# liquidcronos/Drone-stabilisation-using-Optical-Flow-Gps-and-Inertial-Sensors

Measured on AMD Instinct MI355X. Metric: frame-pairs/sec @1920x1080 (LK+velocity), higher is better.
Workload: dtype u8/i32 image stages, f32 LK solve, f64 velocity solve; 1 GPU; 1920x1080 frame pairs, 500 Shi-Tomasi corners, 3-level LK pyramid (BASELINE configs[1]); streams_per_gpu=1, win=15, max_level=3

## Files before the change

drone-stabilisation-using-optical-flow-gps-and-inertial-sensors_amd/csrc/k_corners.hip:

```cpp
#include "ofk_internal.h"
#include <type_traits>

__device__ __forceinline__ int reflect101(int i, int n)
{
    if (n == 1) return 0;
    while (i < 0 || i >= n) i = i < 0 ? -i : 2 * (n - 1) - i;
    return i;
}

#define ME_OW 64
#define ME_CAND_MAX 1920

__device__ __forceinline__ int hs_phys(int x) { return (x & ~7) | ((x & 7) ^ ((x >> 3) & 7)); }

template <int BS, bool FUSED>
__global__ __launch_bounds__(256) void k_mineig(const uint8_t *__restrict__ gray, size_t gray_stride, int h, int w,
                                                int bs_rt, int OH, float kd, float ko, float *__restrict__ eig,
                                                size_t eig_stride, unsigned int *__restrict__ maxbits,
                                                const uint8_t *__restrict__ mask, size_t mask_stride, double quality,
                                                unsigned long long *__restrict__ cand, int cand_cap,
                                                int *__restrict__ cand_count, int *__restrict__ flags)
{
    extern __shared__ __attribute__((aligned(16))) uint8_t smem[];
    const int bs = BS ? BS : bs_rt;
// ... 510 lines not shown
    apc = a + c;
    return __float_as_int(apc - sqrt_rn_normal(__builtin_fmaf(4.f, y2, amc2)));
}

#define OFK_PAIR_SPILL_KEYS()                                                                                          \
    {                                                                                                                  \
        const int nchunk = cnt >> 6;                                                                                   \
        for (int q = 0; q < nchunk; ++q) {                                                                             \
            const unsigned long long key = buf[q * 64 + lane];                                                         \
            if (written + q * 64 + lane < seg_cap) myseg[written + q * 64 + lane] = key;                               \
        }                                                                                                              \
        written += nchunk * 64;                                                                                        \
        const unsigned long long rest = buf[nchunk * 64 + lane];                                                       \
        __builtin_amdgcn_wave_barrier();                                                                               \
        buf[lane] = rest;                                                                                              \
        cnt -= nchunk * 64;                                                                                            \
    }
#define OFK_RING_READ(i)                                                                                               \
        const auto oyye = s_ring[(4 * (i)) * 64 + lane], oyyo = s_ring[(4 * (i) + 1) * 64 + lane];                     \
        const auto oxye = s_ring[(4 * (i) + 2) * 64 + lane], oxyo = s_ring[(4 * (i) + 3) * 64 + lane];
#define OFK_PAIR_ROWS(IN)                                                                                             \
    _Pragma("unroll") for (int i = 0; i < BS; ++i) {                                                                   \
        const int r = base + i;                                                                                        \
        int ge2 = (int)__builtin_amdgcn_ubfe((unsigned)curv[i], bsh, 8u), go2 = (int)__builtin_amdgcn_ubfe((unsigned)curv[i], bsh + 8u, 8u); \
        if (!(IN)) {                                                                                                   \
            if (edge_strip) { ge2 = __builtin_amdgcn_ds_bpermute(mir_e, ge2); go2 = __builtin_amdgcn_ds_bpermute(mir_o, go2); } \
        }                                                                                                              \
        if (i > 0 && (i & 1) == 0 && cnt >= 64) OFK_PAIR_SPILL_KEYS()                                                  \
        OFK_RING_READ(i)                                            \
        const int r12e = g1e + ge2, r12o = g1o + go2;               \
        const int se = r01e + r12e, so = r01o + r12o, te = r12e - r01e, to = r12o - r01o;    \
        const int nso = -so, nse = -se, tt = te + to;                                                                  \
        const int dxe = DPP_SHR1(nso) + so;                                                                            \
        const int dxo = DPP_SHL1(se) + nse;                                                                            \
        int uye = DPP_SHR1(to) + te, uyo = DPP_SHL1(te) + to;    \
        asm("" : "+v"(uye), "+v"(uyo));                                \
        const int dye = uye + tt;                                                                                      \
        const int dyo = uyo + tt;                                                                                      \
        int hxxe, hxxo, hxye, hxyo, hyye, hyyo;                                                                        \
        int pxxe = __mul24(dxe, dxe), pyye = __mul24(dye, dye), pxye = __mul24(dxe, dye);                          \
        int pxxo = __mul24(dxo, dxo), pyyo = __mul24(dyo, dyo), pxyo = __mul24(dxo, dyo);                          \
        asm("" : "+v"(pxxe), "+v"(pxye), "+v"(pyye), "+v"(pxxo), "+v"(pxyo), "+v"(pyyo));                          \
        if (!(IN)) {                                                                                               \
            const int Y = Yp0 + r - 2;                                                                             \
            const bool rowflip = (Y < 0) | (Y >= h);                                                               \
            pxye = (rowflip != flip_e) ? -pxye : pxye;                                                             \
            pxyo = (rowflip != flip_o) ? -pxyo : pxyo;                                                             \
        }                                                                                                          \
        box_pair<BS / 2>(pxxe, pxxo, ad2, ad3, hxxe, hxxo);                                                        \
        box_pair<BS / 2>(pxye, pxyo, ad2, ad3, hxye, hxyo);                                                        \
        box_pair<BS / 2>(pyye, pyyo, ad2, ad3, hyye, hyyo);                                                        \
        vxxe += hxxe - rxxe[i]; vxye += hxye - oxye; vyye += hyye - oyye;                                              \
        vxxo += hxxo - rxxo[i]; vxyo += hxyo - oxyo; vyyo += hyyo - oyyo;                                              \
        rxxe[i] = hxxe; rxxo[i] = hxxo;                                                                                \
        s_ring[(4 * i) * 64 + lane] = hyye; s_ring[(4 * i + 1) * 64 + lane] = hyyo;                                    \
        s_ring[(4 * i + 2) * 64 + lane] = hxye; s_ring[(4 * i + 3) * 64 + lane] = hxyo;                                \
        const int yo = ya - 2 + r - BS;                                                                                \
        const int e2e = lambda_min_bits(vxxe, vxye, vyye, kdv), e2o = lambda_min_bits(vxxo, vxyo, vyyo, kdv);    \
        OFK_PAIR_ROW_TAIL(IN)                                                                                          \
        r01e = r12e; r01o = r12o; g1e = ge2; g1o = go2;                                                                  \
    }
#define OFK_PAIR_ROWS_F32(IN)                                                                                          \
    _Pragma("unroll") for (int i = 0; i < BS; ++i) {                                                                   \
        const int r = base + i;                                                                                        \
        const unsigned gw_ = (unsigned)curv[i] >> bsh;                                                                 \
        float ge2 = (float)(gw_ & 255u), go2 = (float)((gw_ >> 8) & 255u);                                             \
        asm("" : "+v"(ge2), "+v"(go2));                   \
        if (!(IN)) {                                                                                                   \
            if (edge_strip) { ge2 = bperm_f(mir_e, ge2); go2 = bperm_f(mir_o, go2); }                                   \
        }                                                                                                              \
        if (i > 0 && (i & 1) == 0 && cnt >= 64) OFK_PAIR_SPILL_KEYS()                                                  \
        OFK_RING_READ(i)                                                                                               \
        const float r12e = g1e + ge2, r12o = g1o + go2;                                                                \
        const float se = r01e + r12e, so = r01o + r12o, te = r12e - r01e, to = r12o - r01o, tt = te + to;              \
        float dxe = so - DPP_SHR1F(so), dxo = DPP_SHL1F(se) - se;                                                      \
        const float dye = (DPP_SHR1F(to) + te) + tt, dyo = (DPP_SHL1F(te) + to) + tt;                                  \
        if (!(IN)) {                                                                                                   \
            const int Y = Yp0 + r - 2;                                                                                 \
            const bool rowflip = (Y < 0) | (Y >= h);                                                                   \
            dxe = (rowflip != flip_e) ? -dxe : dxe;                                                                    \
            dxo = (rowflip != flip_o) ? -dxo : dxo;                                                                    \
        }                                                                                                              \
        const float gx = bperm_f(adk, dxo), gy = bperm_f(adk, dyo);                                                    \
        float hxxe, hxxo, hxye, hxyo, hyye, hyyo;                                                                      \
        const float pxxe = dxe * dxe, pxye = dxe * dye, pyye = dye * dye;                                              \
        box_pair_f<BS / 2>(pxxe, __builtin_fmaf(dxo, dxo, pxxe), gx, gx, ad2, hxxe, hxxo);                              \
        box_pair_f<BS / 2>(pxye, __builtin_fmaf(dxo, dyo, pxye), gx, gy, ad2, hxye, hxyo);                              \
        box_pair_f<BS / 2>(pyye, __builtin_fmaf(dyo, dyo, pyye), gy, gy, ad2, hyye, hyyo);                              \
// ... 24 lines not shown
        const int hm2e = max(max(DPP_SHR1(e2o), e2e), e2o);                                                         \
        const int hm2o = max(max(DPP_SHL1(e2e), e2o), e2e);                                                         \
        const int yn = yo - 1;                                                                                         \
        const int me = max(max(hm0e, hm1e), hm2e), mo = max(max(hm0o, hm1o), hm2o);                                    \
        bool ise = e1e >= max(me, thr1e), iso = e1o >= max(mo, thr1o);                                                 \
        if (!(IN)) {                                                                                                   \
            const bool rnms = (yn >= ya) & (yn < yb) & (yn >= 1) & (yn < h - 1);                                       \
            ise = ise & rnms; iso = iso & rnms;                                                                        \
        }                                                                                                              \
        if (MASK) {                                                                                                    \
            const uint8_t *mrow = mk + (size_t)min(max(yn, 0), h - 1) * w;                                             \
            ise = ise & (mrow[xoc_e] != 0); iso = iso & (mrow[xoc_o] != 0);                                            \
        }                                                                                                              \
        const unsigned long long bale = __builtin_amdgcn_ballot_w64(ise), balo = __builtin_amdgcn_ballot_w64(iso);     \
        const int ne = (int)__popcll(bale);                                                                            \
        OFK_PAIR_KEY_STORE()                                                                                           \
        cnt += ne + (int)__popcll(balo);                                                                               \
        e1e = e2e; e1o = e2o; hm0e = hm1e; hm0o = hm1o; hm1e = hm2e; hm1o = hm2o;

template <int BS> struct pair_geom {
    static constexpr int AN = BS / 2, PAD = (2 + AN + 3) & ~3, D = PAD - 2 - AN, SW = (125 - BS) & ~3;
};

template <int BS, bool MASK>
__global__ __launch_bounds__(64) __attribute__((amdgpu_waves_per_eu(3, 8))) void k_mineig_pair(
    const uint8_t *__restrict__ gray, size_t gray_stride, int h, int w, int rows_per_strip, float kd, float ko,
    unsigned int *__restrict__ maxbits, const uint8_t *__restrict__ mask, size_t mask_stride, double quality,
    unsigned long long *__restrict__ seg, int seg_cap, int *__restrict__ seg_count, int *__restrict__ flags)
{
    static_assert(BS == 3 || BS == 5 || BS == 7, "pair sums are written for odd boxes up to 7");
    constexpr int AN = pair_geom<BS>::AN, PAD = pair_geom<BS>::PAD, D = pair_geom<BS>::D, SW = pair_geom<BS>::SW;
    constexpr int L0 = (BS + 1) / 2, L1 = (BS + 1 + SW) / 2;
    constexpr int NBUF = 64 + 2 * SW;
    __shared__ unsigned long long s_buf[NBUF + 64];
    __shared__ int s_ring_mem[4 * BS * 64];
    const int lane = threadIdx.x;
    int bxi = blockIdx.x, byi = blockIdx.y, b = blockIdx.z;
    if ((gridDim.z & 7) == 0) {
        const unsigned per = gridDim.x * gridDim.y, n = blockIdx.z * per + blockIdx.y * gridDim.x + blockIdx.x, k = n >> 3, rem = k % per;
        b = 8 * (int)(k / per) + (int)(n & 7);
        byi = (int)(rem / gridDim.x); bxi = (int)(rem % gridDim.x);
    }
    const int sx = bxi;
    if (sx * SW - D >= w) return;
    const int ya = byi * rows_per_strip, yb = min(h, ya + rows_per_strip);
    const uint8_t *img = gray + (size_t)b * gray_stride;
    const uint8_t *mk = MASK ? mask + (size_t)b * mask_stride : nullptr;
    unsigned long long *buf = s_buf;

    const int G0 = sx * SW - PAD;
    const int ce = G0 + 2 * lane;
    const bool edge_strip = G0 < 0 || G0 + 128 > w;
    const bool flip_e = ce < 0 || ce >= w, flip_o = ce + 1 < 0 || ce + 1 >= w;
    const int xo_e = ce - (BS - 1) + AN, xo_o = xo_e + 1;
    const bool lane_ok = lane >= L0 && lane < L1;
    const bool own_e = lane_ok && xo_e >= 0 && xo_e < w, own_o = lane_ok && xo_o >= 0 && xo_o < w;
    const bool nms_e = lane_ok && xo_e >= 1 && xo_e < w - 1, nms_o = lane_ok && xo_o >= 1 && xo_o < w - 1;
    const int xoc_e = min(max(xo_e, 0), w - 1), xoc_o = min(max(xo_o, 0), w - 1);

    const int Yp0 = ya - 1 - AN;
    const int nsteps = (yb - ya) + BS + 3;
    const int nstrips = (w + D + SW - 1) / SW;
    const int nseg = nstrips * (int)gridDim.y, segid = byi * nstrips + sx;
    unsigned long long *myseg = seg + ((size_t)b * nseg + segid) * seg_cap;

    const int lrow = lane >> 5, lk = lane & 31;
    const unsigned ldoff = (unsigned)min(max(G0 + 4 * lk, 0), w - 4);
    const int srcsel = (lane >> 1) * 4;
    const unsigned bsh = (unsigned)(lane & 1) * 16u;
    auto mirror = [&](int c) -> int { c = c < 0 ? -c : c; c = c >= w ? 2 * (w - 1) - c : c; return min(max((c - G0) >> 1, 0), 63) * 4; };
    const int mir_e = mirror(ce), mir_o = mirror(ce + 1);
    const int ad2 = ((lane - 2) & 63) * 4, ad3 = ((lane - 3) & 63) * 4;
    constexpr int NL = (BS + 1) / 2;
    auto row_of = [&](int r) -> int {
        int gy = Yp0 - 1 + min(r, nsteps - 1);
        gy = gy < 0 ? -gy : gy;
        return gy >= h ? 2 * (h - 1) - gy : gy;
    };
#define OFK_PAIR_LOAD(R0, OUT)                                                                                         \
    _Pragma("unroll") for (int q_ = 0; q_ < NL; ++q_) {                                                                \
        const unsigned a_ = (unsigned)row_of((R0) + 2 * q_) * (unsigned)w, b_ = (unsigned)row_of((R0) + 2 * q_ + 1) * (unsigned)w; \
        OUT[q_] = (int)*reinterpret_cast<const unsigned *>(img + ((lrow ? b_ : a_) + ldoff));                          \
    }

    float kdv = kd;
    asm volatile("" : "+v"(kdv));
    const int adk = ((lane - AN) & 63) * 4;
    const float lim = kd * 16776960.f;
    auto march = [&](auto fp) -> bool {
        constexpr bool FP = decltype(fp)::value;
        using T = typename std::conditional<FP, float, int>::type;
        T *const s_ring = reinterpret_cast<T *>(s_ring_mem);
        int written = 0, cnt = 0;
        int lmaxi = 0;
        float published = 0.f;
        unsigned mb_seen = __hip_atomic_load(maxbits + b * OFK_MAX_STRIDE, __ATOMIC_RELAXED, __HIP_MEMORY_SCOPE_AGENT);
        float thr = (float)((double)__uint_as_float(mb_seen) * quality);
        T r01e = 0, r01o = 0, g1e = 0, g1o = 0;
        T rxxe[BS], rxxo[BS];
#pragma unroll
        for (int i = 0; i < BS; ++i) { rxxe[i] = rxxo[i] = 0; }
#pragma unroll
        for (int i = 0; i < 4 * BS; ++i) s_ring[i * 64 + lane] = 0;
        T vxxe = 0, vxye = 0, vyye = 0, vxxo = 0, vxyo = 0, vyyo = 0;
        int e1e = 0, e1o = 0, hm0e = 0, hm0o = 0, hm1e = 0, hm1o = 0;
        unsigned long long inexact = 0;
        int nextg[NL];
        OFK_PAIR_LOAD(0, nextg)

        for (int base = 0; base < nsteps; base += BS) {
            int curv[BS];
#pragma unroll
            for (int i = 0; i < BS; ++i) curv[i] = __builtin_amdgcn_ds_bpermute(srcsel + 128 * (i & 1), nextg[i >> 1]);
            if constexpr (FP) {
                if (inexact) return false;
            }
            {
                unsigned cur_seen = (unsigned)__builtin_amdgcn_readfirstlane((int)mb_seen);
                if (__float_as_uint(published) > cur_seen) cur_seen = __float_as_uint(published);
                thr = (float)((double)__uint_as_float(cur_seen) * quality);
            }
            if (cnt >= 64) {
                OFK_PAIR_SPILL_KEYS()
                const float mw = wave_max_f32(lane_ok ? __int_as_float(lmaxi) : 0.f);
                if (mw > published) {
                    if (lane == 0) (void)atomicMax(maxbits + b * OFK_MAX_STRIDE, __float_as_uint(mw));
                    published = mw;
                }
                mb_seen = __hip_atomic_load(maxbits + b * OFK_MAX_STRIDE, __ATOMIC_RELAXED, __HIP_MEMORY_SCOPE_AGENT);
            }
            OFK_PAIR_LOAD(base + BS, nextg)
            const int r1 = base + BS - 1;
            const bool interior = !edge_strip && Yp0 + base - 2 >= 0 && Yp0 + r1 - 2 < h && base >= BS + 3 && ya - 3 + base - BS >= 1 &&
                                  ya - 2 + r1 - BS < yb && ya - 3 + r1 - BS < h - 1;
            const int thrb = __float_as_int(fmaxf(thr, 0.f)) + 1;
            const int thr1e = nms_e ? thrb : 0x7fffffff, thr1o = nms_o ? thrb : 0x7fffffff;
            if constexpr (FP) {
                if (interior) { OFK_PAIR_ROWS_F32(true) } else { OFK_PAIR_ROWS_F32(false) }
            } else {
                if (interior) { OFK_PAIR_ROWS(true) } else { OFK_PAIR_ROWS(false) }
            }
        }
        if constexpr (FP) {
            if (inexact) return false;
        }
        __builtin_amdgcn_wave_barrier();
        for (int i = lane; i < cnt; i += 64)
            if (written + i < seg_cap) myseg[written + i] = buf[i];
        if (lane == 0) {
            seg_count[(size_t)b * nseg + segid] = min(written + cnt, seg_cap);
            if (written + cnt > seg_cap) (void)atomicOr(flags, 1);
        }
        const float mw = wave_max_f32(lane_ok ? __int_as_float(lmaxi) : 0.f);
        if (lane == 0 && mw > published) (void)atomicMax(maxbits + b * OFK_MAX_STRIDE, __float_as_uint(mw));
        return true;
    };
    if (!march(std::true_type{})) march(std::false_type{});
}

#undef OFK_PAIR_LOAD
#undef OFK_PAIR_ROWS
#undef OFK_PAIR_ROWS_F32
#undef OFK_PAIR_ROW_TAIL
#undef OFK_RING_READ
#undef OFK_PAIR_SPILL_KEYS
#undef OFK_LOAD_BLOCK
#undef OFK_EIG_ROWS

static bool pair_ok(int w, int block)
{
    return !g_ofk_tuning.no_pair && (block == 3 || block == 5 || block == 7) && (w & 3) == 0 && w >= 64;
}
static void pair_sw(int block, int *sw, int *d)
{
    switch (block) {
        case 3: *sw = pair_geom<3>::SW; *d = pair_geom<3>::D; break;
        case 5: *sw = pair_geom<5>::SW; *d = pair_geom<5>::D; break;
        default: *sw = pair_geom<7>::SW; *d = pair_geom<7>::D; break;
    }
}

void ofk_stream_geometry(int h, int w, int block, int batch, int *rows, int *nseg, int *seg_cap)
{
// ... 15 lines not shown
{
    constexpr int SW = 61 - BS;
    int rows, nseg, seg_cap;
    ofk_stream_geometry(h, w, BS, batch, &rows, &nseg, &seg_cap);
    if ((size_t)nseg * seg_cap > seg_keys_per_image || nseg > seg_count_cap) return -1;
    const int strips = (w + SW - 1) / SW;
    const double scale = 1.0 / (4.0 * BS * 255.0);
    const float kd = (float)(0.5 * scale * scale), ko = (float)(scale * scale);
    dim3 grid(strips, (h + rows - 1) / rows, batch);
    if (mask)
        hipLaunchKernelGGL((k_mineig_stream<BS, true>), grid, dim3(256 / 4), 0, s, gray, gray_stride, h, w, rows, kd, ko, maxbits, mask,
                           mask_stride, quality, seg, seg_cap, seg_count, flags);
    else
        hipLaunchKernelGGL((k_mineig_stream<BS, false>), grid, dim3(256 / 4), 0, s, gray, gray_stride, h, w, rows, kd, ko, maxbits, mask,
                           mask_stride, quality, seg, seg_cap, seg_count, flags);
    *nseg_out = nseg; *segcap_out = seg_cap;
    return 0;
}

template <int BS>
static int launch_mineig_pair(hipStream_t s, const uint8_t *gray, size_t gray_stride, int h, int w, unsigned int *maxbits,
                              const uint8_t *mask, size_t mask_stride, double quality, unsigned long long *seg,
                              size_t seg_keys_per_image, int *seg_count, int seg_count_cap, int *flags, int batch, int *nseg_out,
                              int *segcap_out)
{
    constexpr int SW = pair_geom<BS>::SW, D = pair_geom<BS>::D;
    int rows, nseg, seg_cap;
    ofk_stream_geometry(h, w, BS, batch, &rows, &nseg, &seg_cap);
    if ((size_t)nseg * seg_cap > seg_keys_per_image || nseg > seg_count_cap) return -1;
    const int strips = (w + D + SW - 1) / SW;
    const double scale = 1.0 / (4.0 * BS * 255.0);
    const float kd = (float)(0.5 * scale * scale), ko = (float)(scale * scale);
    if (ko != 2.f * kd) return -1;
    dim3 grid(strips, (h + rows - 1) / rows, batch);
    if (mask)
        hipLaunchKernelGGL((k_mineig_pair<BS, true>), grid, dim3(64), 0, s, gray, gray_stride, h, w, rows, kd, ko, maxbits, mask,
                           mask_stride, quality, seg, seg_cap, seg_count, flags);
    else
        hipLaunchKernelGGL((k_mineig_pair<BS, false>), grid, dim3(64), 0, s, gray, gray_stride, h, w, rows, kd, ko, maxbits, mask,
                           mask_stride, quality, seg, seg_cap, seg_count, flags);
    *nseg_out = nseg; *segcap_out = seg_cap;
    return 0;
}

int ofk_launch_mineig_cand(hipStream_t s, const uint8_t *gray, size_t gray_stride, int h, int w, int block,
                           unsigned int *maxbits, const uint8_t *mask, size_t mask_stride, double quality,
                           unsigned long long *cand, int cand_cap, int *cand_count, unsigned long long *seg,
                           size_t seg_keys_per_image, int *seg_count, int seg_count_cap, int *flags, int batch, int *nseg_out,
                           int *segcap_out)
{
    *nseg_out = 0; *segcap_out = 0;
#define ME_ARGS s, gray, gray_stride, h, w, block, nullptr, 0, maxbits, mask, mask_stride, quality, cand, cand_cap, cand_count, flags, batch
#define ST_ARGS s, gray, gray_stride, h, w, maxbits, mask, mask_stride, quality, seg, seg_keys_per_image, seg_count, seg_count_cap, flags, batch, nseg_out, segcap_out
    if (pair_ok(w, block)) {
        switch (block) {
            case 3: return launch_mineig_pair<3>(ST_ARGS);
            case 5: return launch_mineig_pair<5>(ST_ARGS);
            default: return launch_mineig_pair<7>(ST_ARGS);
        }
    }
    switch (block) {
        case 3: return launch_mineig_stream<3>(ST_ARGS);
        case 5: return launch_mineig_stream<5>(ST_ARGS);
        case 7: return launch_mineig_stream<7>(ST_ARGS);
        case 12: return launch_mineig_stream<12>(ST_ARGS);
        default: return launch_mineig_t<0, true>(ME_ARGS);
    }
#undef ST_ARGS
#undef ME_ARGS
}

__global__ __launch_bounds__(256) void k_maxbits(const float *__restrict__ eig, size_t eig_stride,
                                                 const uint8_t *__restrict__ mask, size_t mask_stride, int npx,
                                                 unsigned int *__restrict__ maxbits)
{
    const int b = blockIdx.y;
    const float *e = eig + (size_t)b * eig_stride;
    const uint8_t *mk = mask ? mask + (size_t)b * mask_stride : nullptr;
    float m = 0.f;
    for (int i = blockIdx.x * 256 + threadIdx.x; i < npx; i += gridDim.x * 256)
        if (!mk || mk[i]) m = fmaxf(m, e[i]);
// ... 527 lines not shown
```

drone-stabilisation-using-optical-flow-gps-and-inertial-sensors_amd/csrc/ofk_api.hip:

```cpp
#include "ofk_internal.h"
#include <cmath>
#include <stdarg.h>
#include <stdio.h>
#include <stdlib.h>
#include <string.h>

static char g_create_err[512] = "";

int ofk_fail(ofk_ctx *ctx, int code, const char *fmt, ...)
{
    char *dst = ctx ? ctx->errmsg : g_create_err;
    va_list ap;
    va_start(ap, fmt);
    vsnprintf(dst, 512, fmt, ap);
    va_end(ap);
    return code;
}

#define TRY(expr) do { int rc_ = (expr); if (rc_ != OFK_OK) return rc_; } while (0)
static size_t up(size_t v, size_t a) { return (v + a - 1) / a * a; }

ofk_levels ofk_make_levels(int h, int w, int win, int max_level)
{
    ofk_levels lv;
// ... 114 lines not shown
    c->lk_seed_mode = OFK_SEED_OFF; c->lk_seed_gain = 1.0;
    c->robust = ofk_robust{OFK_ROBUST_OFF, 4.685, 5, 64, 0ull, 0};
    c->gate = ofk_track_gate{OFK_FB_OFF, 0.5, -1, 0.0};
    bool ok = hipEventCreateWithFlags(&c->ev_fork, hipEventDisableTiming) == hipSuccess &&
              hipEventCreateWithFlags(&c->ev_x, hipEventDisableTiming) == hipSuccess;
    for (int k = 0; k < OFK_MAX_STREAMS && ok; ++k)
        ok = hipEventCreateWithFlags(&c->ev_g0[k], hipEventDisableTiming) == hipSuccess &&
             hipEventCreateWithFlags(&c->ev_aux[k], hipEventDisableTiming) == hipSuccess &&
             hipEventCreateWithFlags(&c->ev_lkdone[0][k], hipEventDisableTiming) == hipSuccess &&
             hipEventCreateWithFlags(&c->ev_lkdone[1][k], hipEventDisableTiming) == hipSuccess &&
             hipEventCreateWithFlags(&c->ev_end[k], hipEventDisableTiming) == hipSuccess &&
             hipEventCreateWithFlags(&c->ev_stagger[k], hipEventDisableTiming) == hipSuccess;
    if (!ok) {
        ofk_fail(nullptr, OFK_E_HIP, "hipEventCreate failed");
        ofk_destroy(c);
        return OFK_E_HIP;
    }
    const size_t B = (size_t)max_batch;
    for (int k = 0; k < 2; ++k) { ALLOC(c->bgr[k], B * c->bgr_stride); ALLOC(c->pyr[k], B * c->pyr_stride); }
    ALLOC(c->eig, B * c->img_stride * sizeof(float));
    ALLOC(c->cand, B * (size_t)c->cand_cap * 8);
    c->seg_keys = (size_t)(c->P / 4) + (size_t)(c->P / 4) / 2 + 64 * OFK_SEG_MAX;
    ALLOC(c->cand_seg, B * c->seg_keys * 8);
    ALLOC(c->seg_count, B * OFK_SEG_MAX * 4);
    ALLOC(c->cand_count, B * OFK_CNT_STRIDE * 4); ALLOC(c->maxbits, B * OFK_MAX_STRIDE * 4);
    ALLOC(c->sel_hist, B * 1024 * 4);
    ALLOC(c->sel_keys, B * OFK_CHUNK * 8);
    ALLOC(c->pts_prev, B * max_pts * 8); ALLOC(c->pts_next, B * max_pts * 8);
    ALLOC(c->status, B * max_pts); ALLOC(c->err, B * max_pts * 4); ALLOC(c->counts, B * 4);
    ALLOC(c->sensors, B * OFK_SENSOR_DOUBLES * 8); ALLOC(c->records, B * OFK_RECORD_DOUBLES * 8);
    ALLOC(c->dev_flags, 16);
    hipMemsetAsync(c->dev_flags, 0, 16, c->stream);
    hipMemsetAsync(c->counts, 0, B * 4, c->stream);
    hipMemsetAsync(c->sensors, 0, B * OFK_SENSOR_DOUBLES * 8, c->stream);
    c->ev_cap = 32768;
    c->ev = (hipEvent_t *)calloc(c->ev_cap, sizeof(hipEvent_t));
    c->ev_stage = (int *)calloc(c->ev_cap / 2, sizeof(int));
    hipStreamSynchronize(c->stream);
    *out = c;
    return OFK_OK;
}

extern "C" int ofk_destroy(ofk_ctx *c)
{
    if (!c) return OFK_OK;
    hipSetDevice(c->device);
    if (c->stream) hipDeviceSynchronize();
    ofk_comm_destroy(c);
    for (int k = 0; k < 2; ++k) { if (c->bgr[k]) hipFree(c->bgr[k]); if (c->pyr[k]) hipFree(c->pyr[k]); }
    void *ptrs[] = {c->eig, c->mask, c->deriv, c->cand, c->cand_seg, c->seg_count, c->cand_count, c->sel_hist, c->sel_keys, c->maxbits, c->pts_prev, c->pts_next, c->status, c->err,
                    c->counts, c->sensors, c->records, c->dev_flags, c->scratch, c->pts_new, c->new_counts, c->limit,
                    c->imu_state, c->imu_dv, c->kf_mats, c->kf_x, c->kf_P, c->fused, c->imu_msgs, c->imu_counts, c->rob_work, c->pts_back};
    for (void *p : ptrs) if (p) hipFree(p);
    if (c->hstage) hipHostFree(c->hstage);
    ofk_jpeg_release(c);
    if (c->ev) { for (int i = 0; i < c->ev_cap; ++i) if (c->ev[i]) hipEventDestroy(c->ev[i]); free(c->ev); }
    free(c->ev_stage);
    free(c->h_counts);
    for (int k = 1; k < OFK_MAX_STREAMS; ++k) if (c->streams[k]) hipStreamDestroy(c->streams[k]);
    for (int k = 0; k < OFK_MAX_STREAMS; ++k) {
        if (c->aux[k]) hipStreamDestroy(c->aux[k]);
        if (c->ev_g0[k]) hipEventDestroy(c->ev_g0[k]);
        if (c->ev_aux[k]) hipEventDestroy(c->ev_aux[k]);
        for (int s = 0; s < 2; ++s) if (c->ev_lkdone[s][k]) hipEventDestroy(c->ev_lkdone[s][k]);
    }
    for (int k = 0; k < 2; ++k) if (c->pyr_alt[k]) hipFree(c->pyr_alt[k]);
    for (int k = 0; k < 8; ++k) if (c->marks[k]) hipEventDestroy(c->marks[k]);
    for (int k = 0; k < OFK_MAX_STREAMS; ++k) {
        if (c->ev_end[k]) hipEventDestroy(c->ev_end[k]);
        if (c->ev_stagger[k]) hipEventDestroy(c->ev_stagger[k]);
    }
    if (c->ev_x) hipEventDestroy(c->ev_x);
    if (c->ev_fork) hipEventDestroy(c->ev_fork);
// ... 163 lines not shown
    TRY(check_geom(c, batch, h, w, "ofk_mineig_response"));
    if (!gray || !eig) return ofk_fail(c, OFK_E_INVALID, "ofk_mineig_response: NULL buffer");
    TRY(check_block(c, h, w, block));
    const size_t px = (size_t)h * w;
    TRY(h2d(c, c->pyr[0], c->pyr_stride, gray, px, batch));
    if (ofk_launch_mineig(c->stream, c->pyr[0], c->pyr_stride, h, w, block, c->eig, c->img_stride, nullptr, nullptr, 0, batch))
        return ofk_fail(c, OFK_E_INVALID, "k_mineig: LDS tile too large for block_size %d", block);
    TRY(check_launch(c, "k_mineig"));
    return d2h(c, eig, c->eig, c->img_stride * 4, px * 4, batch);
}

static int check_select(ofk_ctx *c, int max_corners, double quality, double min_distance)
{
    if (max_corners < 1 || max_corners > c->max_pts) return ofk_fail(c, OFK_E_INVALID, "max_corners %d outside 1..%d", max_corners, c->max_pts);
    if (!(quality > 0.0) || !(min_distance >= 0.0)) return ofk_fail(c, OFK_E_INVALID, "quality must be > 0 and min_distance >= 0");
    return OFK_OK;
}

static uint8_t *const *pyr_set(ofk_ctx *c, int set) { return set ? c->pyr_alt : c->pyr; }

struct View {
    int nb;
    uint8_t *bgr[2], *pyr[2];
    unsigned int *maxbits; int *cand_count; unsigned long long *cand, *cand_seg; int *seg_count;
    int nseg, segcap;
    unsigned *sel_hist; unsigned long long *sel_keys;
    float *pts_prev, *pts_next; uint8_t *status; float *err; int *counts;
    double *sensors, *records;
    float *pts_back, *err_back, *fb2; uint8_t *status_back; int *gate_stats;
};
static View view_of(ofk_ctx *c, int b0, int nb, int set)
{
    const size_t b = (size_t)b0;
    uint8_t *const *pyr = pyr_set(c, set);
    View v;
    v.nb = nb;
    for (int k = 0; k < 2; ++k) { v.bgr[k] = c->bgr[k] + b * c->bgr_stride; v.pyr[k] = pyr[k] + b * c->pyr_stride; }
    v.maxbits = c->maxbits + b * OFK_MAX_STRIDE; v.cand_count = c->cand_count + b * OFK_CNT_STRIDE;
    v.cand = c->cand + b * c->cand_cap; v.cand_seg = c->cand_seg + b * c->seg_keys; v.seg_count = c->seg_count + b * OFK_SEG_MAX;
    v.nseg = v.segcap = 0;
    v.sel_hist = c->sel_hist + b * 1024; v.sel_keys = c->sel_keys + b * OFK_CHUNK;
    v.pts_prev = c->pts_prev + b * c->max_pts * 2; v.pts_next = c->pts_next + b * c->max_pts * 2;
    v.status = c->status + b * c->max_pts; v.err = c->err + b * c->max_pts; v.counts = c->counts + b;
    v.sensors = c->sensors + b * OFK_SENSOR_DOUBLES; v.records = c->records + b * OFK_RECORD_DOUBLES;
    v.pts_back = v.err_back = v.fb2 = nullptr; v.status_back = nullptr; v.gate_stats = nullptr;
    if (c->pts_back) {
        v.pts_back = c->pts_back + b * c->max_pts * 2; v.err_back = c->err_back + b * c->max_pts; v.fb2 = c->fb2 + b * c->max_pts;
        v.status_back = c->status_back + b * c->max_pts; v.gate_stats = c->gate_stats + b * 4;
    }
    return v;
}

static int detect_response(ofk_ctx *c, hipStream_t s, View &v, const uint8_t *dmask, int h, int w, int block, double quality)
{
    ofk_launch_zero_detect_state(s, v.maxbits, v.cand_count, v.sel_hist, v.nb);
    if (ofk_launch_mineig_cand(s, v.pyr[0], c->pyr_stride, h, w, block, v.maxbits, dmask, dmask ? c->img_stride : 0, quality, v.cand, c->cand_cap,
                               v.cand_count, v.cand_seg, c->seg_keys, v.seg_count, OFK_SEG_MAX, c->dev_flags, v.nb, &v.nseg, &v.segcap))
        return ofk_fail(c, OFK_E_INVALID, "corner response: block_size %d does not fit (LDS tile / key segments)", block);
    return OFK_OK;
}
static void detect_select(ofk_ctx *c, hipStream_t s, const View &v, int h, int w, int max_corners, double quality, double min_distance,
                          float *dst, int *dst_counts, const int *limit)
{
    ofk_launch_select(s, v.cand, c->cand_cap, v.cand_count, v.cand_seg, v.segcap, v.seg_count, v.nseg, v.maxbits, quality, h, w, max_corners,
                      (float)min_distance, dst, c->max_pts, dst_counts, limit, v.nb, v.sel_hist, v.sel_keys);
}

static int run_select(ofk_ctx *c, const uint8_t *dmask, int batch, int h, int w, int max_corners, double quality, double min_distance)
{
    const View v = view_of(c, 0, batch, 0);
    ofk_launch_zero_detect_state(c->stream, v.maxbits, v.cand_count, v.sel_hist, batch);
    ofk_launch_maxbits(c->stream, c->eig, c->img_stride, dmask, c->img_stride, h, w, v.maxbits, batch);
    ofk_launch_nms(c->stream, c->eig, c->img_stride, dmask, c->img_stride, h, w, v.maxbits, quality, v.cand, c->cand_cap, v.cand_count,
                   c->dev_flags, batch);
    detect_select(c, c->stream, v, h, w, max_corners, quality, min_distance, v.pts_prev, v.counts, nullptr);
    return check_launch(c, "corner selection");
}

static int check_capacity(ofk_ctx *c, const int *flags, int *counts, int batch)
{
// ... 1314 lines not shown
```

drone-stabilisation-using-optical-flow-gps-and-inertial-sensors_amd/csrc/ofk_internal.h:

```cpp
#pragma once
#include <hip/hip_runtime.h>
#include <stdint.h>
#include <stddef.h>
#include "ofk.h"

#define OFK_MAX_LEVELS 9
#define OFK_MAX_STREAMS 8
#define OFK_CHUNK 4096
#define OFK_SEG_MAX 2048
#define OFK_MAX_STRIDE 128
#define OFK_CNT_STRIDE 32

struct ofk_levels {
    int n;
    int h[OFK_MAX_LEVELS], w[OFK_MAX_LEVELS];
    size_t off[OFK_MAX_LEVELS];
};

struct ofk_comm;
struct ofk_ctx {
    int device;
    ofk_comm *comm;
    hipStream_t stream;
    hipStream_t streams[OFK_MAX_STREAMS]; int nstreams;
    hipEvent_t ev_fork;
    hipStream_t aux[OFK_MAX_STREAMS]; int overlap;
    hipEvent_t ev_g0[OFK_MAX_STREAMS], ev_aux[OFK_MAX_STREAMS];
    uint8_t *pyr_alt[2]; int pyr_set;
    int pyr_last;
    hipEvent_t ev_lkdone[2][OFK_MAX_STREAMS];
    hipEvent_t marks[8];
    int slices_open, open_slices;
    hipEvent_t ev_end[OFK_MAX_STREAMS];
    hipEvent_t ev_stagger[OFK_MAX_STREAMS];
    hipEvent_t ev_x; int x_pending;
    int max_w, max_h, max_batch, max_pts, max_level;
    size_t P;
    size_t bgr_stride;
    size_t pyr_stride;
    size_t img_stride;
    int cand_cap;

    uint8_t *bgr[2];
    int gray_direct_set;
    uint8_t *pyr[2];
    float *eig;
    uint8_t *mask;
    int16_t *deriv;
    unsigned long long *cand;
    unsigned long long *cand_seg;
    int *seg_count;
    size_t seg_keys;
    int *cand_count;
    unsigned *sel_hist;
    unsigned long long *sel_keys;
    unsigned int *maxbits;
    float *pts_prev, *pts_next;
    uint8_t *status;
    float *err;
    int *counts;
    float *pts_new;
    int *new_counts, *limit;
    int stream_h, stream_w, stream_batch;
    int *h_counts;
    double *sensors;
    double *records;
    int *dev_flags;
    void *scratch; size_t scratch_bytes;
    void *hstage; size_t hstage_bytes;
    void *jstage;

    double *imu_state, *imu_dv;
    double *kf_mats, *kf_x, *kf_P;
    double *fused;
// ... 35 lines not shown
int ofk_jpeg_decode_device(ofk_ctx *c, const uint8_t *const *jpeg, const size_t *nbytes, int batch, uint8_t *dst, size_t dst_stride,
                           size_t dst_capacity_px, int *h_out, int *w_out, uint8_t **out, size_t *out_stride);

void ofk_launch_gray(hipStream_t s, const uint8_t *bgr, size_t bgr_stride, uint8_t *gray, size_t gray_stride, int batch,
                     int h, int w);
void ofk_launch_pyr_down(hipStream_t s, const uint8_t *src, size_t src_stride, int h, int w, uint8_t *dst,
                         size_t dst_stride, int batch);
void ofk_launch_pyr_down2(hipStream_t s, const uint8_t *src0, const uint8_t *src1, size_t src_stride, int h, int w,
                          uint8_t *dst0, uint8_t *dst1, size_t dst_stride, int batch);
bool ofk_launch_pyr3(hipStream_t s, uint8_t *pyr0, uint8_t *pyr1, size_t stride, const ofk_levels &lv, int batch, int images);
void ofk_launch_scharr(hipStream_t s, const uint8_t *src, size_t src_stride, int h, int w, int16_t *dxdy,
                       size_t dst_stride_elems, int batch);
int  ofk_launch_mineig(hipStream_t s, const uint8_t *gray, size_t gray_stride, int h, int w, int block, float *eig,
                       size_t eig_stride, unsigned int *maxbits, const uint8_t *mask, size_t mask_stride, int batch);
void ofk_launch_maxbits(hipStream_t s, const float *eig, size_t eig_stride, const uint8_t *mask, size_t mask_stride,
                        int h, int w, unsigned int *maxbits, int batch);
void ofk_launch_nms(hipStream_t s, const float *eig, size_t eig_stride, const uint8_t *mask, size_t mask_stride, int h,
                    int w, const unsigned int *maxbits, double quality, unsigned long long *cand, int cand_cap,
                    int *cand_count, int *flags, int batch);
int  ofk_launch_mineig_cand(hipStream_t s, const uint8_t *gray, size_t gray_stride, int h, int w, int block,
                            unsigned int *maxbits, const uint8_t *mask, size_t mask_stride, double quality,
                            unsigned long long *cand, int cand_cap, int *cand_count, unsigned long long *seg,
                            size_t seg_keys_per_image, int *seg_count, int seg_count_cap, int *flags, int batch, int *nseg_out,
                            int *segcap_out);
void ofk_stream_geometry(int h, int w, int block, int batch, int *rows, int *nseg, int *seg_cap);
void ofk_launch_select(hipStream_t s, unsigned long long *cand, int cand_cap, int *cand_count, const unsigned long long *seg,
                       int seg_cap, const int *seg_count, int nseg, const unsigned int *maxbits, double quality, int h, int w,
                       int max_corners, float min_distance, float *pts, int pts_stride, int *counts, const int *limit, int batch,
                       unsigned *sel_hist, unsigned long long *sel_keys);
void ofk_launch_zero_detect_state(hipStream_t s, unsigned int *maxbits, int *cand_count, unsigned *sel_hist, int batch);
void ofk_launch_disc_mask(hipStream_t s, uint8_t *mask, size_t mask_stride, int h, int w, const float *pts, const int *counts,
                          int pts_stride, int radius, const int *limit, int batch);
void ofk_launch_redetect_limits(hipStream_t s, const int *counts, int min_feat, int max_feat, int *limit, int batch);
void ofk_launch_update_tracks(hipStream_t s, const float *next_pts, const uint8_t *status, const int *counts_in, int pts_stride,
                              const float *new_pts, const int *new_counts, float *tracks, int *counts_out, int max_total, int batch);
void ofk_launch_lk(hipStream_t s, const uint8_t *prev, const uint8_t *next, size_t pyr_stride, const ofk_levels &lv,
                   const float *prev_pts, const int *counts, int pts_stride, int win, int max_count, double eps,
                   double min_eig_thr, float *next_pts, uint8_t *status, float *err, int batch, int flags = 0);
void ofk_launch_seed_points(hipStream_t s, const float *pts, const int *counts, int pts_stride, const double *sensors,
                            const double *imu_state, int mode, double gain, float *seed_out, int batch);
void ofk_launch_track_gate(hipStream_t s, const float *prev_pts, const float *back_pts, const uint8_t *st_back, const float *err,
                           const int *counts, int pts_stride, int fb_on, float thr2, int err_on, float err_max, uint8_t *status, float *fb2,
                           int *stats, int batch);
void ofk_launch_pairs_solve(hipStream_t s, const float *prev_pts, const float *next_pts, const uint8_t *status,
                            const int *counts, int pts_stride, const double *sensors, int variant, int use_feas,
                            double feas_T, const int *cand_count, double *records, int batch);
void ofk_launch_pairs_robust(hipStream_t s, const float *prev_pts, const float *next_pts, const uint8_t *status, const int *counts,
// ... 54 lines not shown
```

Measured before the change: 137,200 frame-pairs/s.

## Split float/int mineig march into main kernel plus deferred integer redo kernel

The pair min-eigenvalue kernel used to run the float march and, on inexact results, the integer march inside one kernel, so both code paths inflated register pressure. The float path now runs alone in the main kernel, which also raises its waves-per-EU hint for the unmasked case. Strips that hit inexactness are queued through an atomic counter into a redo list, and a second small kernel reprocesses them with the integer path. The cost is an extra kernel launch on every call and a dependence on the redo counter slot in cand_count being zeroed beforehand.

```diff
diff --git a/drone-stabilisation-using-optical-flow-gps-and-inertial-sensors_amd/csrc/k_corners.hip b/drone-stabilisation-using-optical-flow-gps-and-inertial-sensors_amd/csrc/k_corners.hip
--- a/drone-stabilisation-using-optical-flow-gps-and-inertial-sensors_amd/csrc/k_corners.hip
+++ b/drone-stabilisation-using-optical-flow-gps-and-inertial-sensors_amd/csrc/k_corners.hip
@@ -556,7 +556,7 @@
 #define OFK_PAIR_ROWS(IN)                                                                                             \
     _Pragma("unroll") for (int i = 0; i < BS; ++i) {                                                                   \
         const int r = base + i;                                                                                        \
-        int ge2 = (int)__builtin_amdgcn_ubfe((unsigned)curv[i], bsh, 8u), go2 = (int)__builtin_amdgcn_ubfe((unsigned)curv[i], bsh + 8u, 8u); \
+        int ge2 = (int)__builtin_amdgcn_ubfe((unsigned)curv[i], 0u, 8u), go2 = (int)__builtin_amdgcn_ubfe((unsigned)curv[i], 8u, 8u); \
         if (!(IN)) {                                                                                                   \
             if (edge_strip) { ge2 = __builtin_amdgcn_ds_bpermute(mir_e, ge2); go2 = __builtin_amdgcn_ds_bpermute(mir_o, go2); } \
         }                                                                                                              \
@@ -597,7 +597,7 @@
 #define OFK_PAIR_ROWS_F32(IN)                                                                                          \
     _Pragma("unroll") for (int i = 0; i < BS; ++i) {                                                                   \
         const int r = base + i;                                                                                        \
-        const unsigned gw_ = (unsigned)curv[i] >> bsh;                                                                 \
+        const unsigned gw_ = (unsigned)curv[i];                                                                        \
         float ge2 = (float)(gw_ & 255u), go2 = (float)((gw_ >> 8) & 255u);                                             \
         asm("" : "+v"(ge2), "+v"(go2));                   \
         if (!(IN)) {                                                                                                   \
@@ -668,11 +668,12 @@
     static constexpr int AN = BS / 2, PAD = (2 + AN + 3) & ~3, D = PAD - 2 - AN, SW = (125 - BS) & ~3;
 };
 
-template <int BS, bool MASK>
-__global__ __launch_bounds__(64) __attribute__((amdgpu_waves_per_eu(3, 8))) void k_mineig_pair(
-    const uint8_t *__restrict__ gray, size_t gray_stride, int h, int w, int rows_per_strip, float kd, float ko,
+template <int BS, bool MASK, bool FP>
+__device__ __forceinline__ bool mineig_pair_strip(
+    const uint8_t *__restrict__ gray, size_t gray_stride, int h, int w, int rows_per_strip, float kd,
     unsigned int *__restrict__ maxbits, const uint8_t *__restrict__ mask, size_t mask_stride, double quality,
-    unsigned long long *__restrict__ seg, int seg_cap, int *__restrict__ seg_count, int *__restrict__ flags)
+    unsigned long long *__restrict__ seg, int seg_cap, int *__restrict__ seg_count, int *__restrict__ flags,
+    int b, int byi, int sx, int nchunks)
 {
     static_assert(BS == 3 || BS == 5 || BS == 7, "pair sums are written for odd boxes up to 7");
     constexpr int AN = pair_geom<BS>::AN, PAD = pair_geom<BS>::PAD, D = pair_geom<BS>::D, SW = pair_geom<BS>::SW;
@@ -681,14 +682,6 @@
     __shared__ unsigned long long s_buf[NBUF + 64];
     __shared__ int s_ring_mem[4 * BS * 64];
     const int lane = threadIdx.x;
-    int bxi = blockIdx.x, byi = blockIdx.y, b = blockIdx.z;
-    if ((gridDim.z & 7) == 0) {
-        const unsigned per = gridDim.x * gridDim.y, n = blockIdx.z * per + blockIdx.y * gridDim.x + blockIdx.x, k = n >> 3, rem = k % per;
-        b = 8 * (int)(k / per) + (int)(n & 7);
-        byi = (int)(rem / gridDim.x); bxi = (int)(rem % gridDim.x);
-    }
-    const int sx = bxi;
-    if (sx * SW - D >= w) return;
     const int ya = byi * rows_per_strip, yb = min(h, ya + rows_per_strip);
     const uint8_t *img = gray + (size_t)b * gray_stride;
     const uint8_t *mk = MASK ? mask + (size_t)b * mask_stride : nullptr;
@@ -707,13 +700,17 @@
     const int Yp0 = ya - 1 - AN;
     const int nsteps = (yb - ya) + BS + 3;
     const int nstrips = (w + D + SW - 1) / SW;
-    const int nseg = nstrips * (int)gridDim.y, segid = byi * nstrips + sx;
+    const int nseg = nstrips * nchunks, segid = byi * nstrips + sx;
     unsigned long long *myseg = seg + ((size_t)b * nseg + segid) * seg_cap;
 
-    const int lrow = lane >> 5, lk = lane & 31;
-    const unsigned ldoff = (unsigned)min(max(G0 + 4 * lk, 0), w - 4);
-    const int srcsel = (lane >> 1) * 4;
-    const unsigned bsh = (unsigned)(lane & 1) * 16u;
+#define OFK_PAIR_ROLES()                                                                                               \
+    int rl_ = lane;                                                                                                    \
+    asm volatile("" : "+v"(rl_));                                                                                      \
+    const bool lrow = rl_ >= 32;                                                                                       \
+    const unsigned ldoff = (unsigned)min(max(G0 + 4 * (rl_ & 31), 0), w - 4);                                          \
+    const int srcsel = (rl_ >> 1) * 4;                                                                                 \
+    const unsigned bsh = (unsigned)(rl_ & 1) * 16u;                                                                    \
+    (void)srcsel; (void)bsh;
     auto mirror = [&](int c) -> int { c = c < 0 ? -c : c; c = c >= w ? 2 * (w - 1) - c : c; return min(max((c - G0) >> 1, 0), 63) * 4; };
     const int mir_e = mirror(ce), mir_o = mirror(ce + 1);
     const int ad2 = ((lane - 2) & 63) * 4, ad3 = ((lane - 3) & 63) * 4;
@@ -733,78 +730,117 @@
     asm volatile("" : "+v"(kdv));
     const int adk = ((lane - AN) & 63) * 4;
     const float lim = kd * 16776960.f;
-    auto march = [&](auto fp) -> bool {
-        constexpr bool FP = decltype(fp)::value;
-        using T = typename std::conditional<FP, float, int>::type;
-        T *const s_ring = reinterpret_cast<T *>(s_ring_mem);
-        int written = 0, cnt = 0;
-        int lmaxi = 0;
-        float published = 0.f;
-        unsigned mb_seen = __hip_atomic_load(maxbits + b * OFK_MAX_STRIDE, __ATOMIC_RELAXED, __HIP_MEMORY_SCOPE_AGENT);
-        float thr = (float)((double)__uint_as_float(mb_seen) * quality);
-        T r01e = 0, r01o = 0, g1e = 0, g1o = 0;
-        T rxxe[BS], rxxo[BS];
-#pragma unroll
-        for (int i = 0; i < BS; ++i) { rxxe[i] = rxxo[i] = 0; }
-#pragma unroll
-        for (int i = 0; i < 4 * BS; ++i) s_ring[i * 64 + lane] = 0;
-        T vxxe = 0, vxye = 0, vyye = 0, vxxo = 0, vxyo = 0, vyyo = 0;
-        int e1e = 0, e1o = 0, hm0e = 0, hm0o = 0, hm1e = 0, hm1o = 0;
-        unsigned long long inexact = 0;
-        int nextg[NL];
-        OFK_PAIR_LOAD(0, nextg)
-
-        for (int base = 0; base < nsteps; base += BS) {
-            int curv[BS];
-#pragma unroll
-            for (int i = 0; i < BS; ++i) curv[i] = __builtin_amdgcn_ds_bpermute(srcsel + 128 * (i & 1), nextg[i >> 1]);
-            if constexpr (FP) {
-                if (inexact) return false;
-            }
-            {
-                unsigned cur_seen = (unsigned)__builtin_amdgcn_readfirstlane((int)mb_seen);
-                if (__float_as_uint(published) > cur_seen) cur_seen = __float_as_uint(published);
-                thr = (float)((double)__uint_as_float(cur_seen) * quality);
-            }
-            if (cnt >= 64) {
-                OFK_PAIR_SPILL_KEYS()
-                const float mw = wave_max_f32(lane_ok ? __int_as_float(lmaxi) : 0.f);
-                if (mw > published) {
-                    if (lane == 0) (void)atomicMax(maxbits + b * OFK_MAX_STRIDE, __float_as_uint(mw));
-                    published = mw;
-                }
-                mb_seen = __hip_atomic_load(maxbits + b * OFK_MAX_STRIDE, __ATOMIC_RELAXED, __HIP_MEMORY_SCOPE_AGENT);
-            }
-            OFK_PAIR_LOAD(base + BS, nextg)
-            const int r1 = base + BS - 1;
-            const bool interior = !edge_strip && Yp0 + base - 2 >= 0 && Yp0 + r1 - 2 < h && base >= BS + 3 && ya - 3 + base - BS >= 1 &&
-                                  ya - 2 + r1 - BS < yb && ya - 3 + r1 - BS < h - 1;
-            const int thrb = __float_as_int(fmaxf(thr, 0.f)) + 1;
-            const int thr1e = nms_e ? thrb : 0x7fffffff, thr1o = nms_o ? thrb : 0x7fffffff;
-            if constexpr (FP) {
-                if (interior) { OFK_PAIR_ROWS_F32(true) } else { OFK_PAIR_ROWS_F32(false) }
-            } else {
-                if (interior) { OFK_PAIR_ROWS(true) } else { OFK_PAIR_ROWS(false) }
-            }
-        }
+    using T = typename std::conditional<FP, float, int>::type;
+    T *const s_ring = reinterpret_cast<T *>(s_ring_mem);
+    int written = 0, cnt = 0;
+    int lmaxi = 0;
+    float published = 0.f;
+    unsigned mb_seen = __hip_atomic_load(maxbits + b * OFK_MAX_STRIDE, __ATOMIC_RELAXED, __HIP_MEMORY_SCOPE_AGENT);
+    float thr = (float)((double)__uint_as_float(mb_seen) * quality);
+    T r01e = 0, r01o = 0, g1e = 0, g1o = 0;
+    T rxxe[BS], rxxo[BS];
+#pragma unroll
+    for (int i = 0; i < BS; ++i) { rxxe[i] = rxxo[i] = 0; }
+#pragma unroll
+    for (int i = 0; i < 4 * BS; ++i) s_ring[i * 64 + lane] = 0;
+    T vxxe = 0, vxye = 0, vyye = 0, vxxo = 0, vxyo = 0, vyyo = 0;
+    int e1e = 0, e1o = 0, hm0e = 0, hm0o = 0, hm1e = 0, hm1o = 0;
+    unsigned long long inexact = 0;
+    int nextg[NL];
+    { OFK_PAIR_ROLES() OFK_PAIR_LOAD(0, nextg) }
+
+    for (int base = 0; base < nsteps; base += BS) {
+        OFK_PAIR_ROLES()
+        int curv[BS];
+#pragma unroll
+        for (int i = 0; i < BS; ++i) curv[i] = __builtin_amdgcn_ds_bpermute(srcsel + 128 * (i & 1), nextg[i >> 1]) >> bsh;
         if constexpr (FP) {
             if (inexact) return false;
         }
-        __builtin_amdgcn_wave_barrier();
-        for (int i = lane; i < cnt; i += 64)
-            if (written + i < seg_cap) myseg[written + i] = buf[i];
-        if (lane == 0) {
-            seg_count[(size_t)b * nseg + segid] = min(written + cnt, seg_cap);
-            if (written + cnt > seg_cap) (void)atomicOr(flags, 1);
-        }
-        const float mw = wave_max_f32(lane_ok ? __int_as_float(lmaxi) : 0.f);
-        if (lane == 0 && mw > published) (void)atomicMax(maxbits + b * OFK_MAX_STRIDE, __float_as_uint(mw));
-        return true;
-    };
-    if (!march(std::true_type{})) march(std::false_type{});
+        {
+            unsigned cur_seen = (unsigned)__builtin_amdgcn_readfirstlane((int)mb_seen);
+            if (__float_as_uint(published) > cur_seen) cur_seen = __float_as_uint(published);
+            thr = (float)((double)__uint_as_float(cur_seen) * quality);
+        }
+        if (cnt >= 64) {
+            OFK_PAIR_SPILL_KEYS()
+            const float mw = wave_max_f32(lane_ok ? __int_as_float(lmaxi) : 0.f);
+            if (mw > published) {
+                if (lane == 0) (void)atomicMax(maxbits + b * OFK_MAX_STRIDE, __float_as_uint(mw));
+                published = mw;
+            }
+            mb_seen = __hip_atomic_load(maxbits + b * OFK_MAX_STRIDE, __ATOMIC_RELAXED, __HIP_MEMORY_SCOPE_AGENT);
+        }
+        OFK_PAIR_LOAD(base + BS, nextg)
+        const int r1 = base + BS - 1;
+        const bool interior = !edge_strip && Yp0 + base - 2 >= 0 && Yp0 + r1 - 2 < h && base >= BS + 3 && ya - 3 + base - BS >= 1 &&
+                              ya - 2 + r1 - BS < yb && ya - 3 + r1 - BS < h - 1;
+        const int thrb = __float_as_int(fmaxf(thr, 0.f)) + 1;
+        const int thr1e = nms_e ? thrb : 0x7fffffff, thr1o = nms_o ? thrb : 0x7fffffff;
+        if constexpr (FP) {
+            if (interior) { OFK_PAIR_ROWS_F32(true) } else { OFK_PAIR_ROWS_F32(false) }
+        } else {
+            if (interior) { OFK_PAIR_ROWS(true) } else { OFK_PAIR_ROWS(false) }
+        }
+    }
+    if constexpr (FP) {
+        if (inexact) return false;
+    }
+    __builtin_amdgcn_wave_barrier();
+    for (int i = lane; i < cnt; i += 64)
+        if (written + i < seg_cap) myseg[written + i] = buf[i];
+    if (lane == 0) {
+        seg_count[(size_t)b * nseg + segid] = min(written + cnt, seg_cap);
+        if (written + cnt > seg_cap) (void)atomicOr(flags, 1);
+    }
+    const float mw = wave_max_f32(lane_ok ? __int_as_float(lmaxi) : 0.f);
+    if (lane == 0 && mw > published) (void)atomicMax(maxbits + b * OFK_MAX_STRIDE, __float_as_uint(mw));
+    return true;
+}
+
+
+template <int BS, bool MASK>
+__global__ __launch_bounds__(64) __attribute__((amdgpu_waves_per_eu(MASK ? 3 : 4, 8))) void k_mineig_pair(
+    const uint8_t *__restrict__ gray, size_t gray_stride, int h, int w, int rows_per_strip, float kd, float ko,
+    unsigned int *__restrict__ maxbits, const uint8_t *__restrict__ mask, size_t mask_stride, double quality,
+    unsigned long long *__restrict__ seg, int seg_cap, int *__restrict__ seg_count, int *__restrict__ flags,
+    int *__restrict__ counters, int *__restrict__ redo_list)
+{
+    int bxi = blockIdx.x, byi = blockIdx.y, b = blockIdx.z;
+    if ((gridDim.z & 7) == 0) {
+        const unsigned per = gridDim.x * gridDim.y, n = blockIdx.z * per + blockIdx.y * gridDim.x + blockIdx.x, k = n >> 3, rem = k % per;
+        b = 8 * (int)(k / per) + (int)(n & 7);
+        byi = (int)(rem / gridDim.x); bxi = (int)(rem % gridDim.x);
+    }
+    if (bxi * pair_geom<BS>::SW - pair_geom<BS>::D >= w) return;
+    if (mineig_pair_strip<BS, MASK, true>(gray, gray_stride, h, w, rows_per_strip, kd, maxbits, mask, mask_stride, quality, seg, seg_cap,
+                                          seg_count, flags, b, byi, bxi, (int)gridDim.y))
+        return;
+    if (threadIdx.x == 0) {
+        const int nseg = (int)(gridDim.x * gridDim.y);
+        const int slot = atomicAdd(counters + b * OFK_CNT_STRIDE + OFK_CNT_REDO, 1);
+        redo_list[(size_t)b * nseg + slot] = byi * (int)gridDim.x + bxi;
+    }
+}
+
+template <int BS, bool MASK>
+__global__ __launch_bounds__(64) __attribute__((amdgpu_waves_per_eu(MASK ? 3 : 4, 8))) void k_mineig_pair_redo(
+    const uint8_t *__restrict__ gray, size_t gray_stride, int h, int w, int rows_per_strip, float kd,
+    unsigned int *__restrict__ maxbits, const uint8_t *__restrict__ mask, size_t mask_stride, double quality,
+    unsigned long long *__restrict__ seg, int seg_cap, int *__restrict__ seg_count, int *__restrict__ flags,
+    const int *__restrict__ counters, const int *__restrict__ redo_list, int nstrips, int nchunks)
+{
+    const int b = blockIdx.y;
+    const int n = min(counters[b * OFK_CNT_STRIDE + OFK_CNT_REDO], nstrips * nchunks);
+    for (int e = blockIdx.x; e < n; e += gridDim.x) {
+        const int segid = min(max(redo_list[(size_t)b * (nstrips * nchunks) + e], 0), nstrips * nchunks - 1);
+        (void)mineig_pair_strip<BS, MASK, false>(gray, gray_stride, h, w, rows_per_strip, kd, maxbits, mask, mask_stride, quality, seg,
+                                                 seg_cap, seg_count, flags, b, segid / nstrips, segid % nstrips, nchunks);
+    }
 }
 
 #undef OFK_PAIR_LOAD
+#undef OFK_PAIR_ROLES
 #undef OFK_PAIR_ROWS
 #undef OFK_PAIR_ROWS_F32
 #undef OFK_PAIR_ROW_TAIL
@@ -866,7 +902,7 @@
 static int launch_mineig_pair(hipStream_t s, const uint8_t *gray, size_t gray_stride, int h, int w, unsigned int *maxbits,
                               const uint8_t *mask, size_t mask_stride, double quality, unsigned long long *seg,
                               size_t seg_keys_per_image, int *seg_count, int seg_count_cap, int *flags, int batch, int *nseg_out,
-                              int *segcap_out)
+                              int *segcap_out, int *counters, int *redo_list)
 {
     constexpr int SW = pair_geom<BS>::SW, D = pair_geom<BS>::D;
     int rows, nseg, seg_cap;
@@ -876,13 +912,20 @@
     const double scale = 1.0 / (4.0 * BS * 255.0);
     const float kd = (float)(0.5 * scale * scale), ko = (float)(scale * scale);
     if (ko != 2.f * kd) return -1;
-    dim3 grid(strips, (h + rows - 1) / rows, batch);
-    if (mask)
+    const int chunks = (h + rows - 1) / rows;
+    dim3 grid(strips, chunks, batch);
+    dim3 rgrid(batch >= 128 ? 8 : 4, batch);
+    if (mask) {
         hipLaunchKernelGGL((k_mineig_pair<BS, true>), grid, dim3(64), 0, s, gray, gray_stride, h, w, rows, kd, ko, maxbits, mask,
-                           mask_stride, quality, seg, seg_cap, seg_count, flags);
-    else
+                           mask_stride, quality, seg, seg_cap, seg_count, flags, counters, redo_list);
+        hipLaunchKernelGGL((k_mineig_pair_redo<BS, true>), rgrid, dim3(64), 0, s, gray, gray_stride, h, w, rows, kd, maxbits, mask,
+                           mask_stride, quality, seg, seg_cap, seg_count, flags, counters, redo_list, strips, chunks);
+    } else {
         hipLaunchKernelGGL((k_mineig_pair<BS, false>), grid, dim3(64), 0, s, gray, gray_stride, h, w, rows, kd, ko, maxbits, mask,
-                           mask_stride, quality, seg, seg_cap, seg_count, flags);
+                           mask_stride, quality, seg, seg_cap, seg_count, flags, counters, redo_list);
+        hipLaunchKernelGGL((k_mineig_pair_redo<BS, false>), rgrid, dim3(64), 0, s, gray, gray_stride, h, w, rows, kd, maxbits, mask,
+                           mask_stride, quality, seg, seg_cap, seg_count, flags, counters, redo_list, strips, chunks);
+    }
     *nseg_out = nseg; *segcap_out = seg_cap;
     return 0;
 }
@@ -891,16 +934,16 @@
                            unsigned int *maxbits, const uint8_t *mask, size_t mask_stride, double quality,
                            unsigned long long *cand, int cand_cap, int *cand_count, unsigned long long *seg,
                            size_t seg_keys_per_image, int *seg_count, int seg_count_cap, int *flags, int batch, int *nseg_out,
-                           int *segcap_out)
+                           int *segcap_out, int *redo_list)
 {
     *nseg_out = 0; *segcap_out = 0;
 #define ME_ARGS s, gray, gray_stride, h, w, block, nullptr, 0, maxbits, mask, mask_stride, quality, cand, cand_cap, cand_count, flags, batch
 #define ST_ARGS s, gray, gray_stride, h, w, maxbits, mask, mask_stride, quality, seg, seg_keys_per_image, seg_count, seg_count_cap, flags, batch, nseg_out, segcap_out
     if (pair_ok(w, block)) {
         switch (block) {
-            case 3: return launch_mineig_pair<3>(ST_ARGS);
-            case 5: return launch_mineig_pair<5>(ST_ARGS);
-            default: return launch_mineig_pair<7>(ST_ARGS);
+            case 3: return launch_mineig_pair<3>(ST_ARGS, cand_count, redo_list);
+            case 5: return launch_mineig_pair<5>(ST_ARGS, cand_count, redo_list);
+            default: return launch_mineig_pair<7>(ST_ARGS, cand_count, redo_list);
         }
     }
     switch (block) {
diff --git a/drone-stabilisation-using-optical-flow-gps-and-inertial-sensors_amd/csrc/ofk_api.hip b/drone-stabilisation-using-optical-flow-gps-and-inertial-sensors_amd/csrc/ofk_api.hip
--- a/drone-stabilisation-using-optical-flow-gps-and-inertial-sensors_amd/csrc/ofk_api.hip
+++ b/drone-stabilisation-using-optical-flow-gps-and-inertial-sensors_amd/csrc/ofk_api.hip
@@ -160,7 +160,7 @@
     ALLOC(c->cand, B * (size_t)c->cand_cap * 8);
     c->seg_keys = (size_t)(c->P / 4) + (size_t)(c->P / 4) / 2 + 64 * OFK_SEG_MAX;
     ALLOC(c->cand_seg, B * c->seg_keys * 8);
-    ALLOC(c->seg_count, B * OFK_SEG_MAX * 4);
+    ALLOC(c->seg_count, B * OFK_SEG_MAX * 4); ALLOC(c->redo_list, B * OFK_SEG_MAX * 4);
     ALLOC(c->cand_count, B * OFK_CNT_STRIDE * 4); ALLOC(c->maxbits, B * OFK_MAX_STRIDE * 4);
     ALLOC(c->sel_hist, B * 1024 * 4);
     ALLOC(c->sel_keys, B * OFK_CHUNK * 8);
@@ -186,7 +186,7 @@
     if (c->stream) hipDeviceSynchronize();
     ofk_comm_destroy(c);
     for (int k = 0; k < 2; ++k) { if (c->bgr[k]) hipFree(c->bgr[k]); if (c->pyr[k]) hipFree(c->pyr[k]); }
-    void *ptrs[] = {c->eig, c->mask, c->deriv, c->cand, c->cand_seg, c->seg_count, c->cand_count, c->sel_hist, c->sel_keys, c->maxbits, c->pts_prev, c->pts_next, c->status, c->err,
+    void *ptrs[] = {c->eig, c->mask, c->deriv, c->cand, c->cand_seg, c->seg_count, c->redo_list, c->cand_count, c->sel_hist, c->sel_keys, c->maxbits, c->pts_prev, c->pts_next, c->status, c->err,
                     c->counts, c->sensors, c->records, c->dev_flags, c->scratch, c->pts_new, c->new_counts, c->limit,
                     c->imu_state, c->imu_dv, c->kf_mats, c->kf_x, c->kf_P, c->fused, c->imu_msgs, c->imu_counts, c->rob_work, c->pts_back};
     for (void *p : ptrs) if (p) hipFree(p);
@@ -396,7 +396,7 @@
 struct View {
     int nb;
     uint8_t *bgr[2], *pyr[2];
-    unsigned int *maxbits; int *cand_count; unsigned long long *cand, *cand_seg; int *seg_count;
+    unsigned int *maxbits; int *cand_count; unsigned long long *cand, *cand_seg; int *seg_count, *redo_list;
     int nseg, segcap;
     unsigned *sel_hist; unsigned long long *sel_keys;
     float *pts_prev, *pts_next; uint8_t *status; float *err; int *counts;
@@ -412,6 +412,7 @@
     for (int k = 0; k < 2; ++k) { v.bgr[k] = c->bgr[k] + b * c->bgr_stride; v.pyr[k] = pyr[k] + b * c->pyr_stride; }
     v.maxbits = c->maxbits + b * OFK_MAX_STRIDE; v.cand_count = c->cand_count + b * OFK_CNT_STRIDE;
     v.cand = c->cand + b * c->cand_cap; v.cand_seg = c->cand_seg + b * c->seg_keys; v.seg_count = c->seg_count + b * OFK_SEG_MAX;
+    v.redo_list = c->redo_list + b * OFK_SEG_MAX;
     v.nseg = v.segcap = 0;
     v.sel_hist = c->sel_hist + b * 1024; v.sel_keys = c->sel_keys + b * OFK_CHUNK;
     v.pts_prev = c->pts_prev + b * c->max_pts * 2; v.pts_next = c->pts_next + b * c->max_pts * 2;
@@ -429,7 +430,7 @@
 {
     ofk_launch_zero_detect_state(s, v.maxbits, v.cand_count, v.sel_hist, v.nb);
     if (ofk_launch_mineig_cand(s, v.pyr[0], c->pyr_stride, h, w, block, v.maxbits, dmask, dmask ? c->img_stride : 0, quality, v.cand, c->cand_cap,
-                               v.cand_count, v.cand_seg, c->seg_keys, v.seg_count, OFK_SEG_MAX, c->dev_flags, v.nb, &v.nseg, &v.segcap))
+                               v.cand_count, v.cand_seg, c->seg_keys, v.seg_count, OFK_SEG_MAX, c->dev_flags, v.nb, &v.nseg, &v.segcap, v.redo_list))
         return ofk_fail(c, OFK_E_INVALID, "corner response: block_size %d does not fit (LDS tile / key segments)", block);
     return OFK_OK;
 }
diff --git a/drone-stabilisation-using-optical-flow-gps-and-inertial-sensors_amd/csrc/ofk_internal.h b/drone-stabilisation-using-optical-flow-gps-and-inertial-sensors_amd/csrc/ofk_internal.h
--- a/drone-stabilisation-using-optical-flow-gps-and-inertial-sensors_amd/csrc/ofk_internal.h
+++ b/drone-stabilisation-using-optical-flow-gps-and-inertial-sensors_amd/csrc/ofk_internal.h
@@ -10,6 +10,7 @@
 #define OFK_SEG_MAX 2048
 #define OFK_MAX_STRIDE 128
 #define OFK_CNT_STRIDE 32
+#define OFK_CNT_REDO 3
 
 struct ofk_levels {
     int n;
@@ -50,6 +51,7 @@
     unsigned long long *cand;
     unsigned long long *cand_seg;
     int *seg_count;
+    int *redo_list;
     size_t seg_keys;
     int *cand_count;
     unsigned *sel_hist;
@@ -131,7 +133,7 @@
                             unsigned int *maxbits, const uint8_t *mask, size_t mask_stride, double quality,
                             unsigned long long *cand, int cand_cap, int *cand_count, unsigned long long *seg,
                             size_t seg_keys_per_image, int *seg_count, int seg_count_cap, int *flags, int batch, int *nseg_out,
-                            int *segcap_out);
+                            int *segcap_out, int *redo_list);
 void ofk_stream_geometry(int h, int w, int block, int batch, int *rows, int *nseg, int *seg_cap);
 void ofk_launch_select(hipStream_t s, unsigned long long *cand, int cand_cap, int *cand_count, const unsigned long long *seg,
                        int seg_cap, const int *seg_count, int nseg, const unsigned int *maxbits, double quality, int h, int w,
```

Measured after the change: 126,700 frame-pairs/s. 0.923x the previous value.
